# shahcompbio/MultiModalMuSig.jl

Measured on AMD Instinct MI355X. Metric: E-step docs/sec, higher is better.
Workload: dtype f64; 1 GPU; LDA K=10 alpha=eta=0.1, 10000 docs x 96 SNV terms (BASELINE configs[1]), nnz(rank 0)=913480, one EM iteration per step; docs_rank0=10000, docs_total=10000, terms=96, topics=10, allreduce=none, comm_nranks=1, devices_visible=1

## Files before the change

multimodalmusig.jl_amd/csrc/dev_math.h:

```cpp
#pragma once
#include <hip/hip_runtime.h>

#define MMM_WAVE 64

__device__ __forceinline__ double dev_digamma_series(double x)
{
    double t = 1.0 / x;
    double psi = log(x) - 0.5 * t;
    t *= t;
    double p = -0.4432598039215686;
    p = fma(p, t, 0.08333333333333333);
    p = fma(p, t, -0.021092796092796094);
    p = fma(p, t, 0.007575757575757576);
    p = fma(p, t, -0.004166666666666667);
    p = fma(p, t, 0.003968253968253968);
    p = fma(p, t, -0.008333333333333333);
    p = fma(p, t, 0.08333333333333333);
    return psi - t * p;
}

__device__ __forceinline__ double dev_digamma_pos(double x);

__device__ __forceinline__ double dev_digamma(double x)
{
    if (x > 0.0 && x < 1e40) return dev_digamma_pos(x);
    double psi = 0.0;
    if (x <= 0.0) { psi -= M_PI / tan(M_PI * x); x = 1.0 - x; }
    if (x < 7.0) {
        int n = 7 - (int)floor(x);
        for (int v = 1; v < n; ++v) psi -= 1.0 / (x + (double)v);
        psi -= 1.0 / x;
        x += (double)n;
    }
    return psi + dev_digamma_series(x);
}

__device__ __forceinline__ double dev_rcp(double x)
{
    double r = __builtin_amdgcn_rcp(x);
    r = fma(fma(-x, r, 1.0), r, r);
    r = fma(fma(-x, r, 1.0), r, r);
    return r;
}

__device__ __forceinline__ double dev_max_raw(double a, double b) { double r; asm("v_max_f64 %0, %1, %2" : "=v"(r) : "v"(a), "v"(b)); return r; }
__device__ __forceinline__ double dev_min_raw(double a, double b) { double r; asm("v_min_f64 %0, %1, %2" : "=v"(r) : "v"(a), "v"(b)); return r; }

__device__ __forceinline__ double dev_div(double a, double b)
{
    double y = __builtin_amdgcn_rcp(b);
    y = fma(fma(-b, y, 1.0), y, y);
    y = fma(fma(-b, y, 1.0), y, y);
    const double q = a * y;
    return fma(fma(-b, q, a), y, q);
}

__device__ __forceinline__ double dev_sqrt(double x)
{
    const double y = __builtin_amdgcn_rsq(x);
    const double g0 = x * y, h0 = 0.5 * y;
    const double r0 = fma(-h0, g0, 0.5);
    const double g1 = fma(g0, r0, g0), h1 = fma(h0, r0, h0);
    const double g2 = fma(fma(-g1, g1, x), h1, g1);
    const double g3 = fma(fma(-g2, g2, x), h1, g2);
    return x == 0.0 ? 0.0 : g3;
}

__device__ __forceinline__ double dev_sqrt_pos(double x)
{
    const double y = __builtin_amdgcn_rsq(x);
    const double g0 = x * y, h0 = 0.5 * y;
    const double r0 = fma(-h0, g0, 0.5);
    const double g1 = fma(g0, r0, g0), h1 = fma(h0, r0, h0);
    const double g2 = fma(fma(-g1, g1, x), h1, g1);
    return fma(fma(-g2, g2, x), h1, g2);
}

#include "mmm_arith.h"
__device__ __forceinline__ double dev_digamma_pos(double x) { return ar_digamma_pos(x); }
__device__ __forceinline__ double dev_digamma_ar(double x) { return (x > 0.0 && x < 1e40) ? ar_digamma_pos(x) : dev_digamma(x); }

__device__ __forceinline__ double dev_log_pos(double x);
__device__ __forceinline__ double dev_log_tab(double x, const double* __restrict__ tab)
{
    const int hi = __double2hiint(x), lo = __double2loint(x);
    if (__builtin_expect((unsigned)(hi - 0x00100000) >= 0x7fe00000u, 0))
        return x > 0.0 ? (hi >= 0x7ff00000 ? x : dev_log_pos(x)) : (x == 0.0 ? -__builtin_inf() : __builtin_nan(""));
    const int e = (hi >> 20) - 1023, j = (hi >> 13) & 127;
    const double m = __hiloint2double((hi & 0x000fffff) | 0x3ff00000, lo);
    const double2 t = *reinterpret_cast<const double2*>(tab + 2 * j);
    const double r = fma(m, t.x, -1.0);
    double p = fma(r, -1.0 / 6.0, 0.2);
    p = fma(p, r, -0.25);
    p = fma(p, r, 1.0 / 3.0);
    p = fma(p, r, -0.5);
    p = fma(p, r, 1.0);
    return fma((double)e, 0.6931471805599453, t.y + p * r);
}

__device__ __forceinline__ double dev_log_pos(double x)
{
    int e = __builtin_amdgcn_frexp_exp(x);
    double m = __builtin_amdgcn_frexp_mant(x);
    const bool lo = m < 0.70710678118654752440;
    m = lo ? m + m : m;
    e = lo ? e - 1 : e;
    const double f = m - 1.0;
    const double s = f * dev_rcp(2.0 + f);
    const double z = s * s;
    double R = 1.479819860511658591e-01;
    R = fma(R, z, 1.531383769920937332e-01);
    R = fma(R, z, 1.818357216161805012e-01);
    R = fma(R, z, 2.222219843214978396e-01);
    R = fma(R, z, 2.857142874366239149e-01);
    R = fma(R, z, 3.999999999940941908e-01);
    R = fma(R, z, 6.666666666666735130e-01);
    R *= z;
    const double hfsq = 0.5 * f * f;
    const double dk = (double)e;
    return fma(dk, 6.93147180369123816490e-01, f - (hfsq - fma(s, hfsq + R, dk * 1.90821492927058770002e-10)));
}

__device__ __forceinline__ double dev_xlogx(double x) { return x == 0.0 ? 0.0 : x * log(x); }

__device__ __forceinline__ double wave_sum(double v)
{
#pragma unroll
    for (int off = 32; off > 0; off >>= 1) v += __shfl_xor(v, off, MMM_WAVE);
    return v;
}
__device__ __forceinline__ double wave_max(double v)
{
#pragma unroll
    for (int off = 32; off > 0; off >>= 1) v = fmax(v, __shfl_xor(v, off, MMM_WAVE));
    return v;
}
__device__ __forceinline__ double wave_bcast(double v, int lane) { return __shfl(v, lane, MMM_WAVE); }
__device__ __forceinline__ double wave_readlane(double v, int lane)
{
    const int lo = __builtin_amdgcn_readlane(__double2loint(v), lane), hi = __builtin_amdgcn_readlane(__double2hiint(v), lane);
    return __hiloint2double(hi, lo);
}

template <int CTRL>
__device__ __forceinline__ double dpp_mov_f64(double v)
{
    int lo = __double2loint(v), hi = __double2hiint(v);
    lo = __builtin_amdgcn_update_dpp(0, lo, CTRL, 0xf, 0xf, true);
    hi = __builtin_amdgcn_update_dpp(0, hi, CTRL, 0xf, 0xf, true);
    return __hiloint2double(hi, lo);
}

__device__ __forceinline__ double wave_max_dpp(double v);
typedef unsigned mmm_u2 __attribute__((ext_vector_type(2)));
__device__ __forceinline__ double rows_sum4(double x)
{
    unsigned lo = (unsigned)__double2loint(x), hi = (unsigned)__double2hiint(x);
    mmm_u2 a = __builtin_amdgcn_permlane32_swap(lo, lo, false, false);
    mmm_u2 b = __builtin_amdgcn_permlane32_swap(hi, hi, false, false);
    const double s = __hiloint2double((int)b.x, (int)a.x) + __hiloint2double((int)b.y, (int)a.y);
    lo = (unsigned)__double2loint(s); hi = (unsigned)__double2hiint(s);
    a = __builtin_amdgcn_permlane16_swap(lo, lo, false, false);
    b = __builtin_amdgcn_permlane16_swap(hi, hi, false, false);
    return __hiloint2double((int)b.x, (int)a.x) + __hiloint2double((int)b.y, (int)a.y);
}

__device__ __forceinline__ double wave_max_dpp(double v)
{
    v = fmax(v, dpp_mov_f64<0xB1>(v));
    v = fmax(v, dpp_mov_f64<0x4E>(v));
    v = fmax(v, dpp_mov_f64<0x141>(v));
    v = fmax(v, dpp_mov_f64<0x140>(v));
    unsigned lo = (unsigned)__double2loint(v), hi = (unsigned)__double2hiint(v);
    mmm_u2 a = __builtin_amdgcn_permlane32_swap(lo, lo, false, false);
    mmm_u2 b = __builtin_amdgcn_permlane32_swap(hi, hi, false, false);
    v = fmax(__hiloint2double((int)b.x, (int)a.x), __hiloint2double((int)b.y, (int)a.y));
    lo = (unsigned)__double2loint(v); hi = (unsigned)__double2hiint(v);
    a = __builtin_amdgcn_permlane16_swap(lo, lo, false, false);
    b = __builtin_amdgcn_permlane16_swap(hi, hi, false, false);
    return fmax(__hiloint2double((int)b.x, (int)a.x), __hiloint2double((int)b.y, (int)a.y));
}

template <int L>
__device__ __forceinline__ double group_sum(double v)
{
    v += dpp_mov_f64<0xB1>(v);
    v += dpp_mov_f64<0x4E>(v);
    v += dpp_mov_f64<0x141>(v);
    v += dpp_mov_f64<0x140>(v);
    if (L >= 32) v += __shfl_xor(v, 16, MMM_WAVE);
    if (L >= 64) v += __shfl_xor(v, 32, MMM_WAVE);
    return v;
}
```

multimodalmusig.jl_amd/csrc/lda_reduce.cuh:

```cuda
struct ReduceArgs {
    const double* partial; const double* llpart; int nslab; int VK;
    double* stats;
    LdaCtl* ctl;
    int t;
    int hist_stride;
    double Nglobal, tol;
    double* ll_hist;
    int do_ll, conv_base, run_tail;
    int p2p; unsigned int p2p_seq; P2PArgs px;
    const double* llpart2; int n_ll, ll_in_k2;
    unsigned long long* ll_cells; unsigned int ll_seq;
};

template <bool RB>
__device__ __forceinline__ void rep_reduce(ReduceArgs& r)
{
    if constexpr (RB) {
        const size_t y = blockIdx.y;
        r.partial += y * r.nslab * r.VK; r.llpart += y * r.nslab; r.stats += y * (r.VK + 16);
        r.ctl += y; r.ll_hist += y * r.hist_stride; r.llpart2 += y * 512;
    }
}

__device__ void lda_pass_tail(const ReduceArgs& r)
{
    int stop = 0;
    if (r.do_ll) {
        const int n = r.ctl->n_hist;
        const double ll = r.stats[r.VK] / r.Nglobal;
        r.ll_hist[n] = ll;
        r.ctl->n_hist = n + 1;
        if (n + 1 - r.conv_base > 10) {
            const double prev = r.ll_hist[n - 1];
            if (fabs(prev - ll) / fabs(ll) < r.tol) { stop = 1; r.ctl->stop = 1; r.ctl->stop_iter = r.t - 1; }
        }
    }
    if (!stop) r.ctl->t = r.t;
    r.ctl->ticket = 0;
}

template <bool P2P>
__device__ __forceinline__ void lda_tail_block(const ReduceArgs& r, int lane)
{
    double v = 0.0;
    const bool from_parts = r.ll_in_k2 && !r.ll_cells;
    if (from_parts && r.do_ll) {
        for (int i = lane; i < r.n_ll; i += 64) v += r.llpart2[i];
        v = wave_sum(v);
    }
    if (lane != 0) return;
    if (from_parts) {
        if (r.do_ll) {
            if (P2P && r.p2p) { p2p_send(r.px, r.p2p_seq, r.VK, v); v = p2p_recv_sum(r.px, r.p2p_seq, r.VK, v); }
            r.stats[r.VK] = v;
        }
    } else if (P2P && r.p2p) r.stats[r.VK] = p2p_recv_sum(r.px, r.p2p_seq, r.VK, r.stats[r.VK]);
    lda_pass_tail(r);
}

template <int KP, int L, bool EARLY = false>
__device__ bool lda_ll_block(const LdaDev& c, const double* __restrict__ gprev, const double* __restrict__ bprev, double* llpart2, int lb, int nlb,
                             double* smem, unsigned long long* cell = nullptr, unsigned int seq = 0, const int stop = 0)
{
    __shared__ double s_w[16];
    const int tid = threadIdx.y * 16 + threadIdx.x, lane = tid & 63, wid = tid >> 6;
    constexpr int G = MMM_WAVE / L;
    const int g = lane / L, l = lane % L;
    const int K = c.K, V = c.V, D = c.D;
    double* sBeta = smem;
    double* myT = smem + (size_t)KP * V + ((size_t)wid * G + g) * KP;
    double* sLog = smem + (size_t)KP * V + (size_t)64 * KP;
    const int wslot = ((int64_t)nlb * 16 * G >= (int64_t)D) ? wid * nlb + lb : lb * 16 + wid, nslots = nlb * 16;
    int base = wslot * G;
    int d = base + g;
    bool valid = d < D;
    double gp = (valid && l < K) ? gprev[(size_t)d * K + l] : (l < K ? 1.0 : 0.0);
    constexpr int PRE = 128 / L;
    const bool dense = L == 16 && (c.dense != nullptr || c.dense16 != nullptr);
    const bool h16 = c.dense16 != nullptr;
    const bool ell = dense || c.ell != nullptr;
    int2 pre[PRE];
    const bool fast = L == 16 && dense && h16 && (int64_t)D * K * 8 < ((int64_t)1 << 32) && (int64_t)D * c.Vp * 2 < ((int64_t)1 << 32);
    unsigned wq[4] = {0u, 0u, 0u, 0u};
    const int lk = l < K ? l : K - 1;
    unsigned dl = valid ? (unsigned)d : 0u;
    if (fast) {
        const unsigned* row = at_byte((const unsigned*)c.dense16, (dl * 16u + (unsigned)l) * (unsigned)(c.Vp >> 4) * 2u);
#pragma unroll
        for (int j = 0; j < 4; ++j) wq[j] = row[j];
    } else if (ell) lda_row_read<L, PRE, false, false, false, false>(c, dense, ell, d, valid, l, V, 0, 0, 0, 0, [&](int j, int w, int n) { pre[j] = make_int2(w, n); });
    int64_t start = (!ell && valid) ? c.doc_ptr[d] : 0;
    int W = (!ell && valid) ? (int)(c.doc_ptr[d + 1] - start) : 0;
    if constexpr (EARLY) {
        const double lt = g_mmm_logtab[tid & (MMM_LOGTAB_N - 1)];
        for (int i = tid; i < KP * V; i += 1024) {
            const int v = i / KP, k = i - v * KP;
            const double b = bprev[(size_t)(k < K ? k : K - 1) * V + v];
            sBeta[i] = (k < K) ? b : 0.0;
        }
        if (tid < MMM_LOGTAB_N) sLog[tid] = lt;
    } else {
        for (int i = tid; i < KP * V; i += 1024) { const int v = i / KP, k = i - v * KP; sBeta[i] = (k < K) ? bprev[(size_t)k * V + v] : 0.0; }
        if (tid < MMM_LOGTAB_N) sLog[tid] = g_mmm_logtab[tid];
    }
    MMM_RSTAMP(lb == 0 && tid == 0, 20);
    __syncthreads();
    if constexpr (EARLY) { if (lda_stop_now(stop)) return true; }
    MMM_RSTAMP(lb == 0 && tid == 0, 21);
    double acc = 0.0;
    if (fast) {
        const int nch = (V + L - 1) / L;
        const int stride = nslots * G;
        const unsigned slp2 = (unsigned)(c.Vp >> 4) * 2u;
        unsigned w[4];
#pragma unroll
        for (int j = 0; j < 4; ++j) w[j] = valid ? wq[j] : 0u;
        for (; base < D; base += stride) {
            const int dn = d + stride;
            const bool validn = base + stride < D && dn < D;
            const unsigned dnl = validn ? (unsigned)dn : dl;
            const double Sp = group_sum<L>(gp);
            lds_wave_sync();
            if (l < KP) myT[l] = (l < K) ? dev_div(gp, Sp) : 0.0;
            lds_wave_sync();
            double tv[KP];
#pragma unroll
            for (int k = 0; k < KP; ++k) tv[k] = myT[k];
            double gpn = *at_byte(gprev, (dnl * (unsigned)K + (unsigned)lk) * 8u);
            {
                const unsigned* row = at_byte((const unsigned*)c.dense16, (dnl * 16u + (unsigned)l) * slp2);
#pragma unroll
                for (int j = 0; j < 4; ++j) wq[j] = row[j];
            }
#pragma unroll
            for (int j = 0; j < 8; ++j) {
                if (j < nch) {
                    const unsigned cq = (j & 1) ? w[j / 2] >> 16 : w[j / 2] & 0xffffu;
                    const bool act = valid && j * L + l < V;
                    acc = lda_ll_term<KP>(tv, sBeta + (size_t)(act ? j * L + l : 0) * KP, act, (double)cq, sLog, acc);
                }
            }
            asm volatile("" : "+v"(acc) :: "memory");
            asm volatile("" : "+v"(gpn) :: "memory");
#pragma unroll
            for (int j = 0; j < 4; ++j) asm volatile("" : "+v"(wq[j]) :: "memory");
            d = dn; valid = validn; dl = dnl;
            gp = (valid && l < K) ? gpn : (l < K ? 1.0 : 0.0);
#pragma unroll
            for (int j = 0; j < 4; ++j) w[j] = valid ? wq[j] : 0u;
        }
    } else if (ell) {
        const int nch = (V + L - 1) / L;
        for (; base < D; base += nslots * G) {
            if (base != wslot * G) {
                d = base + g; valid = d < D;
                gp = (valid && l < K) ? gprev[(size_t)d * K + l] : (l < K ? 1.0 : 0.0);
                lda_row_read<L, PRE, false, false, false, false>(c, dense, ell, d, valid, l, V, 0, 0, 0, 0, [&](int j, int w, int n) { pre[j] = make_int2(w, n); });
            }
            const double Sp = group_sum<L>(gp);
            lds_wave_sync();
            if (l < KP) myT[l] = (l < K) ? dev_div(gp, Sp) : 0.0;
            lds_wave_sync();
            double tv[KP];
#pragma unroll
            for (int k = 0; k < KP; ++k) tv[k] = myT[k];
#pragma unroll
            for (int j = 0; j < PRE; ++j) {
                if (j >= nch) break;
                const int2 t = pre[j];
                const bool act = t.x >= 0;
                acc = lda_ll_term<KP>(tv, sBeta + (size_t)(act ? t.x : 0) * KP, act, (double)t.y, sLog, acc);
            }
        }
    } else
    for (; base < D; base += nslots * G) {
        if (base != wslot * G) {
            d = base + g; valid = d < D;
            gp = (valid && l < K) ? gprev[(size_t)d * K + l] : (l < K ? 1.0 : 0.0);
            start = valid ? c.doc_ptr[d] : 0;
            W = valid ? (int)(c.doc_ptr[d + 1] - start) : 0;
        }
        const int2* __restrict__ tcd = c.tc + start;
        const double Sp = group_sum<L>(gp);
        lds_wave_sync();
        if (l < KP) myT[l] = (l < K) ? dev_div(gp, Sp) : 0.0;
        lds_wave_sync();
        double tv[KP];
#pragma unroll
        for (int k = 0; k < KP; ++k) tv[k] = myT[k];
        int nchmax = (W + L - 1) / L;
        if (G >= 2) nchmax = max(nchmax, __shfl_xor(nchmax, 32, MMM_WAVE));
        if (G >= 4) nchmax = max(nchmax, __shfl_xor(nchmax, 16, MMM_WAVE));
        nchmax = __builtin_amdgcn_readfirstlane(nchmax);
        for (int j = 0; j < nchmax; ++j) {
            const int w = j * L + l;
            const bool act = w < W;
            const int2 t = act ? tcd[w] : make_int2(0, 0);
            acc = lda_ll_term<KP>(tv, sBeta + (size_t)t.x * KP, act, (double)t.y, sLog, acc);
        }
    }
    MMM_RSTAMP(lb == 0 && tid == 0, 22);
    acc = wave_sum(acc);
    if (lane == 0) s_w[wid] = acc;
    __syncthreads();
    MMM_RSTAMP(lb == 0 && tid == 0, 23);
    if (tid == 0) {
        double v = 0.0;
#pragma unroll
        for (int w = 0; w < 16; ++w) v += s_w[w];
        if (cell) cell_store(cell, v, seq); else llpart2[lb] = v;
    }
    return false;
}

__device__ void lda_reduce_block(const ReduceArgs& r)
{
    __shared__ double sm[64][17];
    const int stop_req = lda_stop_request(r.ctl);
    const int tx = threadIdx.x, ty = threadIdx.y;
    const int e = blockIdx.x * 16 + tx;
    double acc = 0.0;
    if (e < r.VK) for (int sl = ty; sl < r.nslab; sl += 64) acc += r.partial[(size_t)sl * r.VK + e];
    if (lda_stop_now(stop_req)) {
        if (r.p2p && blockIdx.x == 0 && tx == 0 && ty == 0) p2p_send(r.px, r.p2p_seq, 0, 0.0);
        return;
    }
    sm[ty][tx] = acc;
    __syncthreads();
    if (ty < 8) {
        double v = 0.0;
#pragma unroll
        for (int j = 0; j < 8; ++j) v += sm[ty * 8 + j][tx];
        sm[ty * 8][tx] = v;
    }
    __syncthreads();
    if (ty == 0 && e < r.VK) {
        double v = 0.0;
#pragma unroll
        for (int j = 0; j < 8; ++j) v += sm[j * 8][tx];
        r.stats[e] = v;
        if (r.p2p) p2p_send(r.px, r.p2p_seq, e, v);
    }
    if (blockIdx.x == 0 && ty >= 4 && ty < 8 && r.ll_cells && r.do_ll) {
        const int lane = (ty * 16 + tx) & 63;
        double v = 0.0;
        v = cells_wait_sum(r.ll_cells, r.n_ll, lane, r.ll_seq, r.ctl);
        v = wave_sum(v);
        if (lane == 0) r.stats[r.VK] = v;
    }
    if (blockIdx.x == 0 && ty == 1 && !r.ll_in_k2 && !r.ll_cells) {
        double v = 0.0;
        for (int i = tx + 16 * 0; i < r.nslab; i += 16) v += r.llpart[i];
        v = group_sum<16>(v);
        if (tx == 0) { r.stats[r.VK] = v; if (r.p2p) p2p_send(r.px, r.p2p_seq, r.VK, v); }
    }
}

template <bool RB = false>
__global__ __launch_bounds__(1024) void k_lda_reduce(ReduceArgs r)
{
    if constexpr (RB) rep_reduce<RB>(r);
    lda_reduce_block(r);
}

template <int KP, bool RB = false>
__global__ __launch_bounds__(1024) void k_lda_reduce_ll(ReduceArgs r, LdaDev c, const double* gprev, const double* bprev, double* llpart2, int nred)
{
    extern __shared__ __attribute__((aligned(16))) double smem[];
    if constexpr (RB) {
        rep_reduce<RB>(r);
        gprev = rep<RB>(gprev, (size_t)c.K * c.D); bprev = rep<RB>(bprev, (size_t)c.V * c.K); llpart2 = rep<RB>(llpart2, 512);
    }
    if ((int)blockIdx.x < nred) { lda_reduce_block(r); return; }
    if (r.ctl->stop) return;
    constexpr int L = KP <= 15 ? 16 : (KP <= 31 ? 32 : 64);
    const int lb = (int)blockIdx.x - nred;
    lda_ll_block<KP, L>(c, gprev, bprev, llpart2, lb, (int)gridDim.x - nred, smem, r.ll_cells ? r.ll_cells + 2 * lb : nullptr, r.ll_seq);
}

struct IldaDesc {
    int I, V, K, SJ;
    int J[kIldaMaxI], joff[kIldaMaxI + 1];
    double eta[kIldaMaxI];
    const int* features;
};

struct IldaMerge {
    IldaDesc ds;
    double* ilam; double* iEln; double* ibeta;
    unsigned long long* fcells;
};

struct MergeArgs {
    int V; double eta;
    Ring lambda, Elnbeta, expElnbeta, beta;
    unsigned long long* cells;
    unsigned int seq;
    int nred;
    int ll_join;
    int n_ll;
    int epb, nredp;
    int pro;
    const double* pro_gamma; double* pro_Eln; double* pro_a;
};

template <int KP, bool P2P, bool ILDA>
__global__ __launch_bounds__(1024) void k_lda_reduce_ll_mstep(ReduceArgs r, LdaDev c, const double* gprev, const double* bprev, MergeArgs ms, IldaMerge im)
{
    extern __shared__ __attribute__((aligned(16))) double smem[];
    __shared__ double sm2[2][64][17];
    asm volatile("" :: "s"(r.ctl), "s"(r.partial), "s"(r.nslab), "s"(r.VK), "s"(c.D), "s"(c.V), "s"(c.K), "s"(c.Vp), "s"(c.doc_ptr), "s"(c.tc), "s"(c.ell),
                 "s"(c.dense), "s"(c.dense16), "s"(gprev), "s"(bprev), "s"(ms.nredp), "s"(ms.nred), "s"(ms.n_ll), "s"(ms.ll_join), "s"(ms.epb), "s"(ms.pro),
                 "s"(ms.pro_gamma), "s"(ms.cells), "s"(ms.seq));
    const int stop_req = lda_stop_request(r.ctl);
    const int tx = threadIdx.x, ty = threadIdx.y, tid = ty * 16 + tx;
    MMM_RSTAMP(blockIdx.x == 1 && tid == 0, 0);
    MMM_RSTAMP(blockIdx.x == 0 && tid == 64, 8);
    MMM_RSTAMP((int)blockIdx.x == ms.nredp && tid == 0, 16);
    if ((int)blockIdx.x >= ms.nredp) {
        constexpr int L = KP <= 15 ? 16 : (KP <= 31 ? 32 : 64);
        const int lb = (int)blockIdx.x - ms.nredp, n_ll = ms.n_ll;
        MMM_LLSTAMP(0, lb);
        double gnx = 0.0;
        int pd = 0;
        if constexpr (KP <= 12) {
            if (ms.pro) {
                const int lane = tid & 63, l = lane & 15;
                pd = ((tid >> 6) * n_ll + lb) * 4 + (lane >> 4);
                gnx = ms.pro_gamma[(size_t)(pd < c.D ? pd : 0) * c.K + (l < c.K ? l : c.K - 1)];
            }
        }
        if (lda_ll_block<KP, L, true>(c, gprev, bprev, nullptr, lb, n_ll + (ms.ll_join ? ms.nredp - 1 : 0), smem, ms.cells + 2 * (ms.nred + lb), ms.seq, stop_req)) return;
        MMM_RSTAMP((int)blockIdx.x == ms.nredp && tid == 0, 17);
        MMM_LLSTAMP(1, lb);
        if constexpr (KP <= 12) {
            if (ms.pro) {
                const int lane = tid & 63, g = lane >> 4, l = lane & 15, K = c.K;
                const double el = lda_elntheta<16>((pd < c.D && l < K) ? gnx : (l < K ? 1.0 : 0.0), g, l, K);
                if (pd < c.D && l < K) { ms.pro_Eln[(size_t)pd * K + l] = el; ms.pro_a[(size_t)pd * K + l] = ar_exp(el); }
            }
        }
        return;
    }
    const int rbp = (int)blockIdx.x, epb = ms.epb;
    const int rb = rbp * epb + (ty < epb ? ty : 0);
    const int e = rb * 16 + tx;
    double acc = 0.0, acc1 = 0.0;
    {
        const int e0 = rbp * epb * 16 + tx;
        if (epb == 2) {
            for (int sl = ty; sl < r.nslab; sl += 64) { acc += r.partial[(size_t)sl * r.VK + e0]; acc1 += r.partial[(size_t)sl * r.VK + e0 + 16]; }
        } else {
            for (int sl = ty; sl < r.nslab; sl += 64) acc += r.partial[(size_t)sl * r.VK + e0];
        }
    }
    if (lda_stop_now(stop_req)) {
        if (P2P && rbp == 0 && tid == 0) { p2p_send(r.px, r.p2p_seq, 0, 0.0); (void)p2p_recv_sum(r.px, r.p2p_seq, 0, 0.0); }
        return;
    }
    MMM_RSTAMP(blockIdx.x == 1 && tid == 0, 1);
    sm2[0][ty][tx] = acc; sm2[1][ty][tx] = acc1;
    __syncthreads();
    if (ty < 8) {
#pragma unroll
        for (int h = 0; h < 2; ++h) {
            double v = 0.0;
#pragma unroll
            for (int j = 0; j < 8; ++j) v += sm2[h][ty * 8 + j][tx];
            sm2[h][ty * 8][tx] = v;
        }
    }
    __syncthreads();
    double (*sm)[17] = sm2[ty < epb ? ty : 0];
    MMM_RSTAMP(blockIdx.x == 1 && tid == 0, 2);
    if (ty < epb) {
        double v = 0.0;
#pragma unroll
        for (int j = 0; j < 8; ++j) v += sm[j * 8][tx];
        if (P2P) { p2p_send(r.px, r.p2p_seq, e, v); v = p2p_recv_sum(r.px, r.p2p_seq, e, v); }
        r.stats[e] = v;
        const int V = ms.V, Vp = (V + 15) & ~15, nb = Vp / 16, k = e / Vp, vv = e - k * Vp, slot = r.t % 3;
        const bool real = vv < V;
        if (ILDA) {
            const IldaDesc& ds = im.ds;
            const int K = ds.K, SJ = ds.SJ;
            int qi = 0, qj = 0;
            double mine = 0.0;
            for (int i = 0; i < ds.I; ++i) {
                const int fi = real ? ds.features[(size_t)i * V + vv] : -1;
                for (int j = 0; j < ds.J[i]; ++j) {
                    const double pq = group_sum<16>(fi == j ? v : 0.0);
                    if (tx == ds.joff[i] + j) { mine = pq; qi = i; qj = j; }
                }
            }
            if (tx < SJ) cell_store(im.fcells + 2 * ((size_t)rb * 16 + tx), mine, ms.seq);
            double lam = 0.0;
            if (tx < SJ) {
                lam = ds.eta[qi];
                for (int b = 0; b < nb; ++b) lam += cell_wait(im.fcells + 2 * ((size_t)(k * nb + b) * 16 + tx), ms.seq, r.ctl);
            }
            double cs = 0.0;
            for (int i = 0; i < ds.I; ++i) {
                const double ci = group_sum<16>((tx < SJ && qi == i) ? lam : 0.0);
                if (tx < SJ && qi == i) cs = ci;
            }
            double el = 0.0, bq = 1.0;
            if (tx < SJ) {
                el = dev_digamma_pos(lam) - dev_digamma_pos(cs); bq = lam / cs;
                if (vv == tx) {
                    const size_t o = (size_t)K * ds.joff[qi] + (size_t)ds.J[qi] * k + qj;
                    im.ilam[o] = lam; im.iEln[o] = el; im.ibeta[o] = bq;
                }
            }
            lds_wave_sync();
            sm[1][tx] = el; sm[2][tx] = bq;
            lds_wave_sync();
            if (real) {
                double ee = 0.0, bb = 1.0;
                for (int i = 0; i < ds.I; ++i) { const int q = ds.joff[i] + ds.features[(size_t)i * V + vv]; ee += sm[1][q]; bb *= sm[2][q]; }
                const size_t o = (size_t)k * V + vv;
                ms.Elnbeta.s[slot][o] = ee; ms.expElnbeta.s[slot][o] = exp(ee); ms.beta.s[slot][o] = bb;
            }
        } else {
        const double lam = real ? ms.eta + v : 0.0;
        const double part = group_sum<16>(lam);
        if (tx == 0) cell_store(ms.cells + 2 * rb, part, ms.seq);
        const double got = (tx < nb) ? cell_wait(ms.cells + 2 * (k * nb + tx), ms.seq, r.ctl) : 0.0;
        double cs = 0.0;
        for (int j = 0; j < nb; ++j) cs += __shfl(got, j, 16);
        MMM_RSTAMP(blockIdx.x == 1 && tid == 0, 3);
        const double el = dev_digamma_pos(real ? lam : 1.0) - dev_digamma_pos(cs);
        const size_t o = (size_t)k * V + vv;
        if (real) { ms.lambda.s[slot][o] = lam; ms.Elnbeta.s[slot][o] = el; ms.expElnbeta.s[slot][o] = exp(el); ms.beta.s[slot][o] = lam / cs; }
        MMM_RSTAMP(blockIdx.x == 1 && tid == 0, 4);
        }
    }
    if (ms.ll_join && rbp > 0) {
        constexpr int L = KP <= 15 ? 16 : (KP <= 31 ? 32 : 64);
        const int n_ll = ms.n_ll, lb = n_ll + rbp - 1;
        lda_ll_block<KP, L>(c, gprev, bprev, nullptr, lb, n_ll + ms.nredp - 1, smem, ms.cells + 2 * (ms.nred + lb), ms.seq);
        return;
    }
    if (rbp == 0 && ty >= 4 && ty < 8) {
        const int lane = tid & 63, n_ll = ms.n_ll + (ms.ll_join ? ms.nredp - 1 : 0);
        const int n = r.ctl->n_hist;
        const double prev = (r.do_ll && n > 0) ? r.ll_hist[n - 1] : 0.0;
        double v = 0.0;
        if (r.do_ll) {
            MMM_RSTAMP(lane == 0, 9);
            v = cells_wait_sum(ms.cells + 2 * ms.nred, n_ll, lane, ms.seq, r.ctl);
            MMM_RSTAMP(lane == 0, 10);
            v = wave_sum(v);
            if (P2P && lane == 0) { p2p_send(r.px, r.p2p_seq, r.VK, v); v = p2p_recv_sum(r.px, r.p2p_seq, r.VK, v); }
        }
        if (lane == 0) {
            int halt = 0;
            if (r.do_ll) {
                r.stats[r.VK] = v;
                const double ll = v / r.Nglobal;
                r.ll_hist[n] = ll;
                r.ctl->n_hist = n + 1;
                if (n + 1 - r.conv_base > 10 && fabs(prev - ll) / fabs(ll) < r.tol) { halt = 1; r.ctl->stop = 1; r.ctl->stop_iter = r.t - 1; }
            }
            if (!halt) r.ctl->t = r.t;
            r.ctl->ticket = 0;
        }
        MMM_RSTAMP(lane == 0, 11);
    }
}

template <bool P2P, bool RB = false>
__global__ __launch_bounds__(128) void k_lda_mstep(ReduceArgs r, int V, double eta, Ring lambda, Ring Elnbeta, Ring expElnbeta, Ring beta)
{
    if constexpr (RB) rep_reduce<RB>(r);
    const int stop = r.ctl->stop;
    const int k = blockIdx.x, tid = threadIdx.x, lane = tid & 63, c = r.t % 3;
    if (k == (int)gridDim.x - 1) {
        if (!stop && tid < 64) lda_tail_block<P2P>(r, lane);
        return;
    }
    double* sums = r.stats + (size_t)k * V;
    if (P2P && r.p2p) {
        if (!stop) for (int v = tid; v < V; v += 128) sums[v] = p2p_recv_sum(r.px, r.p2p_seq, k * V + v, sums[v]);
        else if (k == 0 && tid == 0) (void)p2p_recv_sum(r.px, r.p2p_seq, 0, 0.0);
        __syncthreads();
    }
    double part = 0.0;
    for (int v = lane; v < V; v += 64) part += eta + sums[v];
    if (stop) return;
    const double cs = wave_sum(part);
    const double psi = dev_digamma_pos(cs);
    if constexpr (RB) {
        const size_t VK = (size_t)V * (gridDim.x - 1);
        double* lam = rep<RB>(lambda.s[c], VK); double* Eln = rep<RB>(Elnbeta.s[c], VK); double* eEln = rep<RB>(expElnbeta.s[c], VK); double* bet = rep<RB>(beta.s[c], VK);
        for (int v = tid; v < V; v += 128) {
            const double l = eta + sums[v];
            const double el = dev_digamma_pos(l) - psi;
            const size_t e = (size_t)k * V + v;
            lam[e] = l; Eln[e] = el; eEln[e] = exp(el); bet[e] = l / cs;
        }
        return;
    }
    for (int v = tid; v < V; v += 128) {
        const double l = eta + sums[v];
        const double el = dev_digamma_pos(l) - psi;
        const size_t e = (size_t)k * V + v;
        lambda.s[c][e] = l; Elnbeta.s[c][e] = el; expElnbeta.s[c][e] = exp(el); beta.s[c][e] = l / cs;
    }
}

__global__ __launch_bounds__(512) void k_lda_mstep_wide(ReduceArgs r, int V, double eta, Ring lambda, Ring Elnbeta, Ring expElnbeta, Ring beta)
{
    __shared__ double sh[16];
    const int stop = r.ctl->stop;
    const int k = blockIdx.x, tid = threadIdx.x, lane = tid & 63, wid = tid >> 6, c = r.t % 3;
    if (k == (int)gridDim.x - 1) {
        if (!stop && tid < 64) lda_tail_block<false>(r, lane);
        return;
    }
    if (stop) return;
    const double* sums = r.stats + (size_t)k * V;
    double part = 0.0;
    for (int v = tid; v < V; v += 512) part += eta + sums[v];
    part = wave_sum(part);
    if (lane == 0) sh[wid] = part;
    __syncthreads();
    double cs = 0.0;
#pragma unroll
    for (int w = 0; w < 8; ++w) cs += sh[w];
    const double psi = dev_digamma_pos(cs);
    for (int v = tid; v < V; v += 512) {
        const double l = eta + sums[v];
        const double el = dev_digamma_pos(l) - psi;
        const size_t e = (size_t)k * V + v;
        lambda.s[c][e] = l; Elnbeta.s[c][e] = el; expElnbeta.s[c][e] = exp(el); beta.s[c][e] = l / cs;
    }
}


__global__ __launch_bounds__(64 * kIldaMaxI) void k_ilda_mstep(IldaDesc ds, int mode, const double* sums, double* ilam, double* iEln, double* ibeta,
                                                   double* Eeff, double* expEeff, double* beff, const int* stop, int write_beta_only,
                                                   ReduceArgs tail, int with_tail)
{
    __shared__ double sE[kIldaMaxSJ], sB[kIldaMaxSJ];
    if (stop && *stop) return;
    const int k = blockIdx.x, lane = threadIdx.x & 63, wid = threadIdx.x >> 6, nwv = blockDim.x >> 6, V = ds.V, K = ds.K;
    if (with_tail && k == K) {
        if (wid == 0) lda_tail_block<false>(tail, lane);
        return;
    }
    const bool in_regs = mode == 0 && V <= 256;
    double sv[4] = {0.0, 0.0, 0.0, 0.0};
    if (in_regs) {
#pragma unroll
        for (int q = 0; q < 4; ++q) { const int v = lane + 64 * q; if (v < V) sv[q] = sums[(size_t)k * V + v]; }
    }
    for (int i = wid; i < ds.I; i += nwv) {
        const int Ji = ds.J[i];
        const size_t base = (size_t)K * ds.joff[i] + (size_t)Ji * k;
        const int* f = ds.features + (size_t)i * V;
        int fv[4] = {-1, -1, -1, -1};
        if (in_regs) {
#pragma unroll
            for (int q = 0; q < 4; ++q) { const int v = lane + 64 * q; if (v < V) fv[q] = f[v]; }
        }
        double part = 0.0;
        for (int j0 = 0; j0 < Ji; j0 += 64) {
            const int j = j0 + lane;
            double l = 0.0;
            if (mode == 0) {
                for (int jj = j0; jj < min(Ji, j0 + 64); ++jj) {
                    double t = 0.0;
                    if (in_regs) {
#pragma unroll
                        for (int q = 0; q < 4; ++q) t += (fv[q] == jj) ? sv[q] : 0.0;
                    } else
                        for (int v = lane; v < V; v += 64) t += (f[v] == jj) ? sums[(size_t)k * V + v] : 0.0;
                    t = wave_sum(t);
                    if (lane == jj - j0) l = ds.eta[i] + t;
                }
                if (j < Ji) ilam[base + j] = l;
            } else if (j < Ji) l = ilam[base + j];
            part += l;
        }
        const double cs = wave_sum(part);
        const double psi = dev_digamma_pos(cs);
        for (int j0 = 0; j0 < Ji; j0 += 64) {
            const int j = j0 + lane;
            if (j < Ji) {
                double el, b;
                if (mode == 2) { el = iEln[base + j]; b = ibeta[base + j]; }
                else {
                    const double l = ilam[base + j];
                    el = dev_digamma_pos(l) - psi; b = l / cs;
                    if (!write_beta_only) iEln[base + j] = el;
                    ibeta[base + j] = b;
                }
                sE[ds.joff[i] + j] = el; sB[ds.joff[i] + j] = b;
            }
        }
    }
    __syncthreads();
    for (int v = threadIdx.x; v < V; v += blockDim.x) {
        double e = 0.0, b = 1.0;
        for (int i = 0; i < ds.I; ++i) { const int j = ds.features[(size_t)i * V + v]; e += sE[ds.joff[i] + j]; b *= sB[ds.joff[i] + j]; }
        const size_t o = (size_t)k * V + v;
        if (!write_beta_only) { Eeff[o] = e; expEeff[o] = exp(e); }
        beff[o] = b;
    }
}

__global__ __launch_bounds__(64) void k_lda_infer_tail(ReduceArgs r, int phase)
{
    if (r.ctl->stop) return;
    const int lane = threadIdx.x;
    if (phase & 1) {
        double v = 0.0;
        for (int i = lane; i < r.nslab; i += 64) v += r.llpart[i];
        v = wave_sum(v);
        if (lane == 0) r.stats[r.VK] = v;
    }
    if ((phase & 2) && lane == 0) {
        const int n = r.ctl->n_hist;
        const double ll = r.stats[r.VK] / r.Nglobal;
        r.ll_hist[n] = ll;
        r.ctl->n_hist = n + 1;
        if (n + 1 - r.conv_base > 10) {
            const double prev = r.ll_hist[n - 1];
            if (fabs(prev - ll) / fabs(ll) < r.tol) { r.ctl->stop = 1; r.ctl->stop_iter = r.t; }
        }
        r.ctl->t = r.t;
    }
}

__global__ void k_lda_tail_only(ReduceArgs r) { if (!r.ctl->stop) lda_pass_tail(r); }
```

multimodalmusig.jl_amd/csrc/lda_rows.cuh:

```cuda

__device__ __forceinline__ int row_slot(int w, int slp) { return (w & 15) * slp + (w >> 4); }
__device__ __forceinline__ int row16_count(unsigned w0, unsigned w1, unsigned w2, unsigned w3, int c)
{
    const unsigned word = c < 4 ? (c < 2 ? w0 : w1) : (c < 6 ? w2 : w3);
    return (int)((c & 1) ? word >> 16 : word & 0xffffu);
}

__device__ __forceinline__ void lda_row16_load(const LdaDev& c, const int dl, const int l, unsigned (&w)[4])
{
    const unsigned* __restrict__ r32 = (const unsigned*)(c.dense16 + (size_t)dl * c.Vp + (size_t)l * (c.Vp >> 4));
#pragma unroll
    for (int q = 0; q < 4; ++q) w[q] = r32[q];
}
template <int L, int PRE, bool ROT, bool ZERO_OFF, class Put>
__device__ __forceinline__ void lda_row16_put(const unsigned (&w4)[4], const bool valid, const int l, const int V, const int nch, const int rot, Put&& put)
{
#pragma unroll
    for (int j = 0; j < PRE; ++j) {
        int q = j; if (ROT) { q += rot; if (q >= nch) q -= nch; }
        const int w = q * L + l;
        const bool in = valid && (!ROT || j < nch) && w < V;
        const int n = in ? row16_count(w4[0], w4[1], w4[2], w4[3], q) : 0;
        put(j, (ZERO_OFF ? n > 0 : in) ? w : -1, n);
    }
}

template <int L, int PRE, bool ROT, bool ZERO_OFF, bool WIDE16, bool GROUP, class Put>
__device__ __forceinline__ void lda_row_read(const LdaDev& c, const bool counts, const bool pairs, const int d, const bool valid, const int l, const int V,
                                             const int nch, const int rot, const int64_t start, const int W, Put&& put)
{
    auto chunk = [&](int j) { int q = j; if (ROT) { q += rot; if (q >= nch) q -= nch; } return q; };
    if (counts) {
        const int* __restrict__ row = c.dense + (size_t)(valid ? d : 0) * c.Vp;
        const unsigned short* __restrict__ row16 = c.dense16 + (size_t)(valid ? d : 0) * c.Vp;
        const bool h16 = c.dense16 != nullptr;
        const int slp = c.Vp >> 4;
        if (WIDE16 && L == 16 && h16) {
            unsigned w[4];
            lda_row16_load(c, valid ? d : 0, l, w);
            lda_row16_put<L, PRE, ROT, ZERO_OFF>(w, valid, l, V, nch, rot, put);
        } else if constexpr (!GROUP) {
#pragma unroll
            for (int j = 0; j < PRE; ++j) {
                const int q = chunk(j), w = q * L + l;
                const bool in = valid && (!ROT || j < nch) && w < V;
                const int n = in ? (h16 ? (int)row16[row_slot(w, slp)] : row[row_slot(w, slp)]) : 0;
                put(j, (ZERO_OFF ? n > 0 : in) ? w : -1, n);
            }
        } else {
            int n[PRE];
            if (h16) {
#pragma unroll
                for (int j = 0; j < PRE; ++j) { const int w = chunk(j) * L + l; n[j] = (int)row16[row_slot(w < V ? w : 0, slp)]; }
            } else {
#pragma unroll
                for (int j = 0; j < PRE; ++j) { const int w = chunk(j) * L + l; n[j] = row[row_slot(w < V ? w : 0, slp)]; }
            }
            __builtin_amdgcn_sched_barrier(0);
#pragma unroll
            for (int j = 0; j < PRE; ++j) {
                const int w = chunk(j) * L + l;
                const bool in = valid && (!ROT || j < nch) && w < V;
                const int nn = in ? n[j] : 0;
                put(j, (ZERO_OFF ? nn > 0 : in) ? w : -1, nn);
            }
        }
    } else {
        const int2* __restrict__ src = pairs ? c.ell + (size_t)(valid ? d : 0) * V : c.tc + start;
        const int lim = pairs ? (valid ? V : 0) : W;
        if constexpr (!GROUP) {
#pragma unroll
            for (int j = 0; j < PRE; ++j) {
                const int w = chunk(j) * L + l;
                const int2 p = ((!ROT || j < nch) && w < lim) ? src[w] : make_int2(-1, 0);
                put(j, p.x, p.y);
            }
        } else {
            int2 p[PRE];
#pragma unroll
            for (int j = 0; j < PRE; ++j) {
                const int w = chunk(j) * L + l;
                const int2* __restrict__ at = ((!ROT || j < nch) && w < lim) ? src + w : (const int2*)c.doc_ptr;
                p[j] = *at;
            }
            __builtin_amdgcn_sched_barrier(0);
#pragma unroll
            for (int j = 0; j < PRE; ++j) {
                const int w = chunk(j) * L + l;
                const bool in = (!ROT || j < nch) && w < lim;
                put(j, in ? p[j].x : -1, in ? p[j].y : 0);
            }
        }
    }
}

template <int L>
__device__ __forceinline__ double lda_elntheta(const double gk, const int g, const int l, const int K)
{
    const double S = group_sum<L>(gk);
    const double ps = dev_digamma_pos(l < K ? gk : S);
    return ps - __shfl(ps, g * L + K, MMM_WAVE);
}

template <int KP>
__device__ __forceinline__ double lda_ll_term(const double (&tv)[KP], const double* bc, const bool act, const double count, const double* sLog, const double acc)
{
    double p0 = 0.0, p1 = 0.0;
#pragma unroll
    for (int k = 0; k + 1 < KP; k += 2) { p0 = fma(tv[k], bc[k], p0); p1 = fma(tv[k + 1], bc[k + 1], p1); }
    if (KP & 1) p0 = fma(tv[KP - 1], bc[KP - 1], p0);
    const double p = act ? p0 + p1 : 1.0;
    return fma(count, dev_log_tab(p, sLog), acc);
}
```

Baseline: 640.6 million docs/s.

## Hoist log special-case checks out of LDA log-likelihood inner loop

```diff
diff --git a/multimodalmusig.jl_amd/csrc/dev_math.h b/multimodalmusig.jl_amd/csrc/dev_math.h
--- a/multimodalmusig.jl_amd/csrc/dev_math.h
+++ b/multimodalmusig.jl_amd/csrc/dev_math.h
@@ -81,11 +81,9 @@
 __device__ __forceinline__ double dev_digamma_ar(double x) { return (x > 0.0 && x < 1e40) ? ar_digamma_pos(x) : dev_digamma(x); }
 
 __device__ __forceinline__ double dev_log_pos(double x);
-__device__ __forceinline__ double dev_log_tab(double x, const double* __restrict__ tab)
+__device__ __forceinline__ double dev_log_tab_normal(double x, const double* __restrict__ tab)
 {
     const int hi = __double2hiint(x), lo = __double2loint(x);
-    if (__builtin_expect((unsigned)(hi - 0x00100000) >= 0x7fe00000u, 0))
-        return x > 0.0 ? (hi >= 0x7ff00000 ? x : dev_log_pos(x)) : (x == 0.0 ? -__builtin_inf() : __builtin_nan(""));
     const int e = (hi >> 20) - 1023, j = (hi >> 13) & 127;
     const double m = __hiloint2double((hi & 0x000fffff) | 0x3ff00000, lo);
     const double2 t = *reinterpret_cast<const double2*>(tab + 2 * j);
@@ -96,6 +94,14 @@
     p = fma(p, r, -0.5);
     p = fma(p, r, 1.0);
     return fma((double)e, 0.6931471805599453, t.y + p * r);
+}
+__device__ __forceinline__ bool dev_not_pos_normal(double x) { return __builtin_amdgcn_class(x, 0x2ff); }
+__device__ __forceinline__ double dev_log_tab(double x, const double* __restrict__ tab)
+{
+    const int hi = __double2hiint(x);
+    if (__builtin_expect((unsigned)(hi - 0x00100000) >= 0x7fe00000u, 0))
+        return x > 0.0 ? (hi >= 0x7ff00000 ? x : dev_log_pos(x)) : (x == 0.0 ? -__builtin_inf() : __builtin_nan(""));
+    return dev_log_tab_normal(x, tab);
 }
 
 __device__ __forceinline__ double dev_log_pos(double x)
diff --git a/multimodalmusig.jl_amd/csrc/lda_reduce.cuh b/multimodalmusig.jl_amd/csrc/lda_reduce.cuh
--- a/multimodalmusig.jl_amd/csrc/lda_reduce.cuh
+++ b/multimodalmusig.jl_amd/csrc/lda_reduce.cuh
@@ -59,7 +59,7 @@
 }
 
 template <int KP, int L, bool EARLY = false>
-__device__ bool lda_ll_block(const LdaDev& c, const double* __restrict__ gprev, const double* __restrict__ bprev, double* llpart2, int lb, int nlb,
+__device__ __forceinline__ bool lda_ll_block(const LdaDev& c, const double* __restrict__ gprev, const double* __restrict__ bprev, double* llpart2, int lb, int nlb,
                              double* smem, unsigned long long* cell = nullptr, unsigned int seq = 0, const int stop = 0)
 {
     __shared__ double s_w[16];
@@ -112,13 +112,25 @@
         const int nch = (V + L - 1) / L;
         const int stride = nslots * G;
         const unsigned slp2 = (unsigned)(c.Vp >> 4) * 2u;
+        const bool full = (V & (L - 1)) == 0;
+        const double* bl = sBeta + (size_t)l * KP;
+        int sb = __builtin_amdgcn_readfirstlane(base);
+        unsigned goff = (dl * (unsigned)K + (unsigned)lk) * 8u, roff = (dl * 16u + (unsigned)l) * slp2;
+        const unsigned gstep = (unsigned)stride * (unsigned)K * 8u, rstep = (unsigned)stride * 16u * slp2;
         unsigned w[4];
 #pragma unroll
-        for (int j = 0; j < 4; ++j) w[j] = valid ? wq[j] : 0u;
-        for (; base < D; base += stride) {
+        for (int j = 0; j < 4; ++j) w[j] = wq[j];
+        for (; sb < D; sb += stride) {
             const int dn = d + stride;
-            const bool validn = base + stride < D && dn < D;
-            const unsigned dnl = validn ? (unsigned)dn : dl;
+            const bool validn = dn < D;
+            const unsigned goffn = validn ? goff + gstep : goff, roffn = validn ? roff + rstep : roff;
+            gp = l < K ? gp : 0.0;
+            if (sb + G > D) {
+                asm volatile("");
+                gp = valid ? gp : (l < K ? 1.0 : 0.0);
+#pragma unroll
+                for (int j = 0; j < 4; ++j) w[j] = valid ? w[j] : 0u;
+            }
             const double Sp = group_sum<L>(gp);
             lds_wave_sync();
             if (l < KP) myT[l] = (l < K) ? dev_div(gp, Sp) : 0.0;
@@ -126,28 +138,21 @@
             double tv[KP];
 #pragma unroll
             for (int k = 0; k < KP; ++k) tv[k] = myT[k];
-            double gpn = *at_byte(gprev, (dnl * (unsigned)K + (unsigned)lk) * 8u);
+            double gpn = *at_byte(gprev, goffn);
             {
-                const unsigned* row = at_byte((const unsigned*)c.dense16, (dnl * 16u + (unsigned)l) * slp2);
+                const unsigned* row = at_byte((const unsigned*)c.dense16, roffn);
 #pragma unroll
                 for (int j = 0; j < 4; ++j) wq[j] = row[j];
             }
-#pragma unroll
-            for (int j = 0; j < 8; ++j) {
-                if (j < nch) {
-                    const unsigned cq = (j & 1) ? w[j / 2] >> 16 : w[j / 2] & 0xffffu;
-                    const bool act = valid && j * L + l < V;
-                    acc = lda_ll_term<KP>(tv, sBeta + (size_t)(act ? j * L + l : 0) * KP, act, (double)cq, sLog, acc);
-                }
-            }
+            acc = full ? lda_ll_step16<KP, true>(tv, sBeta, bl, w, valid, l, V, nch, sLog, acc)
+                       : lda_ll_step16<KP, false>(tv, sBeta, bl, w, valid, l, V, nch, sLog, acc);
             asm volatile("" : "+v"(acc) :: "memory");
             asm volatile("" : "+v"(gpn) :: "memory");
 #pragma unroll
             for (int j = 0; j < 4; ++j) asm volatile("" : "+v"(wq[j]) :: "memory");
-            d = dn; valid = validn; dl = dnl;
-            gp = (valid && l < K) ? gpn : (l < K ? 1.0 : 0.0);
-#pragma unroll
-            for (int j = 0; j < 4; ++j) w[j] = valid ? wq[j] : 0u;
+            d = dn; valid = validn; goff = goffn; roff = roffn; gp = gpn;
+#pragma unroll
+            for (int j = 0; j < 4; ++j) w[j] = wq[j];
         }
     } else if (ell) {
         const int nch = (V + L - 1) / L;
diff --git a/multimodalmusig.jl_amd/csrc/lda_rows.cuh b/multimodalmusig.jl_amd/csrc/lda_rows.cuh
--- a/multimodalmusig.jl_amd/csrc/lda_rows.cuh
+++ b/multimodalmusig.jl_amd/csrc/lda_rows.cuh
@@ -112,3 +112,41 @@
     const double p = act ? p0 + p1 : 1.0;
     return fma(count, dev_log_tab(p, sLog), acc);
 }
+
+template <int KP, bool FULL>
+__device__ __forceinline__ double lda_ll_step16(const double (&tv)[KP], const double* sBeta, const double* bl, const unsigned (&w)[4], const bool valid,
+                                                const int l, const int V, const int nch, const double* sLog, const double acc)
+{
+    double a = acc;
+    bool bad = false;
+    int n = __builtin_amdgcn_readfirstlane(nch);
+    asm volatile("" : "+s"(n));
+#pragma unroll
+    for (int j = 0; j < 8; ++j) {
+        if (j < n) {
+            const unsigned cq = (j & 1) ? w[j / 2] >> 16 : w[j / 2] & 0xffffu;
+            const bool act = FULL || (valid && j * 16 + l < V);
+            const double* bc = FULL ? bl + (size_t)j * 16 * KP : sBeta + (size_t)(act ? j * 16 + l : 0) * KP;
+            double p0 = 0.0, p1 = 0.0;
+#pragma unroll
+            for (int k = 0; k + 1 < KP; k += 2) { p0 = fma(tv[k], bc[k], p0); p1 = fma(tv[k + 1], bc[k + 1], p1); }
+            if (KP & 1) p0 = fma(tv[KP - 1], bc[KP - 1], p0);
+            const double p = act ? p0 + p1 : 1.0;
+            bad |= dev_not_pos_normal(p);
+            a = fma((double)cq, dev_log_tab_normal(p, sLog), a);
+        }
+    }
+    if (__builtin_expect(__builtin_amdgcn_ballot_w64(bad) != 0, 0)) {
+        a = acc;
+        asm volatile("" : "+s"(n));
+#pragma unroll
+        for (int j = 0; j < 8; ++j) {
+            if (j < n) {
+                const unsigned cq = (j & 1) ? w[j / 2] >> 16 : w[j / 2] & 0xffffu;
+                const bool act = valid && j * 16 + l < V;
+                a = lda_ll_term<KP>(tv, sBeta + (size_t)(act ? j * 16 + l : 0) * KP, act, (double)cq, sLog, a);
+            }
+        }
+    }
+    return a;
+}
```

Result: faster. 666.4 million docs/s (median of 6 runs) (+4.0%).
